# qcraftai/gedepth

Measured on AMD Instinct MI355X. Metric: training img/s (whole node), KITTI-shaped 352x1120 synthetic batches, higher is better.
Workload: dtype bf16; 1 GPU; depthformer_swint_v: DepthFormer-SwinT + GEDepth-Vanilla, 352x1120, 8 img/GPU, full train step; global_batch=8, parallelism=dp1, allreduce_dtype=fp32, layout=nhwc, window_attention=bf16 mfma, params=53516992, hip_graph=off

## Files before the change

### gedepth_amd/csrc/conv1x1_bn.hip

```cpp
#include "common.h"

#define CB_K 64
#define CB_LD 72
#define CB_GRAM (65 * CB_K)
#define CB_GRAM_WG 256

__device__ __forceinline__ int cb_row(int r, int hi) { return (r & 3) + 8 * (r >> 2) + 4 * hi; }

__global__ void __launch_bounds__(256) conv1x1_gram_k(const bf16_t* __restrict__ x, long rows, float* __restrict__ partial) {
  __shared__ __attribute__((aligned(16))) bf16_t stage_all[4][64 * CB_LD];
  __shared__ float red[CB_GRAM];
  const int lane = threadIdx.x & 63, wv = threadIdx.x >> 6, hi = lane >> 5;
  bf16_t* stage = stage_all[wv];
  ge_f32x16 acc[2][2], sum[2];
#pragma unroll
  for (int i = 0; i < 16; ++i) { acc[0][0][i] = 0.f; acc[0][1][i] = 0.f; acc[1][0][i] = 0.f; acc[1][1][i] = 0.f; sum[0][i] = 0.f; sum[1][i] = 0.f; }
  const ge_bf16x8 ones = {(__bf16)1.f, (__bf16)1.f, (__bf16)1.f, (__bf16)1.f, (__bf16)1.f, (__bf16)1.f, (__bf16)1.f, (__bf16)1.f};
  const int tr_row = hi * 8 + ((lane & 15) >> 2), tr_col = ((lane >> 4) & 1) * 16 + (lane & 3) * 4;
  const long nblk = (rows + 63) / 64;
  for (long blk = (long)blockIdx.x * 4 + wv; blk < nblk; blk += (long)gridDim.x * 4) {
    uint4 R[8];
#pragma unroll
    for (int i = 0; i < 8; ++i) {
      const int idx = i * 64 + lane;
// ... 79 lines not shown
  const int lane = threadIdx.x & 63, wv = threadIdx.x >> 6;
  cb_load_gram(gram, Ss, ss);
  const int c = blockIdx.x * 4 + wv;
  const double wi = c < Cout ? (double)bf2f(w[(long)c * CB_K + lane]) : 0.0;
  ws[wv][lane] = wi;
  __syncthreads();
  double t = 0.0;
#pragma unroll 8
  for (int j = 0; j < CB_K; ++j) t += Ss[lane * 65 + j] * ws[wv][j];
  const double mean = ge_wave_sum(wi * ss[lane]) / n;
  const double ez2 = ge_wave_sum(wi * t) / n;
  if (c >= Cout || lane != 0) return;
  double var = ez2 - mean * mean;
  if (var < 0.0) var = 0.0;
  const float rstd = (float)(1.0 / sqrt(var + (double)eps));
  save_mean[c] = (float)mean;
  save_rstd[c] = rstd;
  if (running_mean) running_mean[c] = (1.f - momentum) * running_mean[c] + momentum * (float)mean;
  if (running_var) running_var[c] = (1.f - momentum) * running_var[c] + momentum * (float)(n > 1.0 ? var * n / (n - 1.0) : var);
  const float a = gamma[c] * rstd;
  coef[c] = a;
  coef[Cout + c] = __fmaf_rn(-(float)mean, a, beta[c]);
}

#ifndef CB_EPI_GROUP
#define CB_EPI_GROUP 4
#endif
#ifdef CB_NT_STORE
#define CB_STORE16(P_, V_) { const uint4 v__ = (V_); __builtin_nontemporal_store((ge_u32x4){v__.x, v__.y, v__.z, v__.w}, (ge_u32x4*)(P_)); }
#else
#define CB_STORE16(P_, V_) *(uint4*)(P_) = (V_)
#endif
#define CB_YLD 136
template <bool HAS_POS>
__global__ void __launch_bounds__(256) conv1x1_bn_act_k(const bf16_t* __restrict__ x, const bf16_t* __restrict__ w, const float* __restrict__ coef,
                                                        const float* __restrict__ pos, bf16_t* __restrict__ y, bf16_t* __restrict__ q,
                                                        long HW, int B, int Cout, float slope) {
  __shared__ __attribute__((aligned(16))) bf16_t ytile_all[4][32 * CB_YLD];
  const int lane = threadIdx.x & 63, wv = threadIdx.x >> 6, hi = lane >> 5, n = lane & 31;
  const int cg = blockIdx.y * 4 + wv;
  if (cg * 128 >= Cout) return;
  bf16_t* ytile = ytile_all[wv];
  const int c0 = cg * 128;
  ge_bf16x8 Wf[4][4];
  float ca[4], cbv[4];
#pragma unroll
  for (int jb = 0; jb < 4; ++jb) {
#pragma unroll
    for (int s = 0; s < 4; ++s) Wf[jb][s] = *(const ge_bf16x8*)(w + (long)(c0 + jb * 32 + n) * CB_K + s * 16 + hi * 8);
    ca[jb] = coef[c0 + jb * 32 + n];
    cbv[jb] = coef[Cout + c0 + jb * 32 + n];
  }
  const int xcd = blockIdx.x & 7, wgx = gridDim.x >> 3, j0 = blockIdx.x >> 3;
  const long npt = (HW + 31) / 32;
  const long npx = npt > xcd ? (npt - xcd + 7) / 8 : 0;
  const long nq = npx * B;
  ge_bf16x8 A[4];
#define CB_LOAD_A(T_)                                                                           \
  {                                                                                             \
    const long pl_ = (T_) / B;                                                                  \
    const int b_ = (int)((T_) - pl_ * B);                                                       \
    const long p_ = (pl_ * 8 + xcd) * 32 + n;                                                   \
    const bf16_t* xr = x + ((long)b_ * HW + (p_ < HW ? p_ : HW - 1)) * CB_K + hi * 8;           \
    _Pragma("unroll") for (int s = 0; s < 4; ++s) A[s] = *(const ge_bf16x8*)(xr + s * 16);      \
  }
  if (j0 < nq) CB_LOAD_A((long)j0)
  for (long t = j0; t < nq; t += wgx) {
    const long pl = t / B;
    const int b = (int)(t - pl * B);
    const long p0 = (pl * 8 + xcd) * 32;
    ge_f32x16 acc[4];
#pragma unroll
    for (int jb = 0; jb < 4; ++jb) {
#pragma unroll
      for (int i = 0; i < 16; ++i) acc[jb][i] = 0.f;
#pragma unroll
      for (int s = 0; s < 4; ++s) acc[jb] = __builtin_amdgcn_mfma_f32_32x32x16_bf16(A[s], Wf[jb][s], acc[jb], 0, 0, 0);
    }
    if (t + wgx < nq) CB_LOAD_A(t + wgx)
    __builtin_amdgcn_wave_barrier();
#pragma unroll
    for (int jb = 0; jb < 4; ++jb)
#pragma unroll
      for (int r = 0; r < 16; ++r) {
        const float z = __fmaf_rn(acc[jb][r], ca[jb], cbv[jb]);
        ytile[cb_row(r, hi) * CB_YLD + jb * 32 + n] = f2bf_hw(z > 0.f ? z : z * slope);
      }
    __builtin_amdgcn_wave_barrier();
#pragma unroll
    for (int i0 = 0; i0 < 8; i0 += CB_EPI_GROUP) {
      float4 e0[CB_EPI_GROUP], e1[CB_EPI_GROUP];
      uint4 v[CB_EPI_GROUP];
      if (HAS_POS) {
#pragma unroll
        for (int i = 0; i < CB_EPI_GROUP; ++i) {
          const int idx = (i0 + i) * 64 + lane, tok = idx >> 4, piece = idx & 15;
          const long pr = p0 + tok < HW ? p0 + tok : HW - 1;
          const float* pp = pos + pr * Cout + c0 + piece * 8;
          e0[i] = *(const float4*)pp;
          e1[i] = *(const float4*)(pp + 4);
        }
      }
#pragma unroll
      for (int i = 0; i < CB_EPI_GROUP; ++i) {
        const int idx = (i0 + i) * 64 + lane, tok = idx >> 4, piece = idx & 15;
        v[i] = *(const uint4*)(ytile + tok * CB_YLD + piece * 8);
        if (p0 + tok < HW) CB_STORE16(y + ((long)b * HW + p0 + tok) * Cout + c0 + piece * 8, v[i]);
      }
      if (HAS_POS) {
#pragma unroll
        for (int i = 0; i < CB_EPI_GROUP; ++i) {
          const int idx = (i0 + i) * 64 + lane, tok = idx >> 4, piece = idx & 15;
          const uint32_t u[4] = {v[i].x, v[i].y, v[i].z, v[i].w};
          const float e[8] = {e0[i].x, e0[i].y, e0[i].z, e0[i].w, e1[i].x, e1[i].y, e1[i].z, e1[i].w};
          uint32_t o[4];
#pragma unroll
          for (int k = 0; k < 4; ++k) {
            const float lo = __uint_as_float(u[k] << 16) + e[2 * k], hi2 = __uint_as_float(u[k] & 0xffff0000u) + e[2 * k + 1];
            o[k] = ge_pack_bf16x2(lo, hi2);
          }
          if (p0 + tok < HW) CB_STORE16(q + ((long)b * HW + p0 + tok) * Cout + c0 + piece * 8, make_uint4(o[0], o[1], o[2], o[3]));
        }
      }
    }
  }
#undef CB_LOAD_A
}

template <bool ONE, bool TWO>
__global__ void __launch_bounds__(256) conv1x1_bn_mask_k(const bf16_t* __restrict__ dy1, long ld1, const bf16_t* __restrict__ dy2, long ld2,
                                                         const bf16_t* __restrict__ y, bf16_t* __restrict__ g, float* __restrict__ partial, int C, long R,
// ... 176 lines not shown
    }
  }
#undef CB_ROWPTR
#undef CB_LOADG
#undef CB_MMA
}

static inline bool cb_ok(int Cin, int Cout) { return Cin == CB_K && Cout > 0 && Cout % 128 == 0 && Cout <= 2048; }

extern "C" size_t ge_conv1x1_bn_workspace(int Cin, int Cout) {
  if (!cb_ok(Cin, Cout)) return 0;
  const size_t a = (size_t)CB_GRAM_WG * CB_GRAM * sizeof(float), b = (size_t)1024 * Cout * sizeof(float);
  return a > b ? a : b;
}

extern "C" int ge_conv1x1_bn_stats(const void* x, long rows, int Cin, const void* w, int Cout, const float* gamma, const float* beta,
                                   float* running_mean, float* running_var, float eps, float momentum, double* gram, float* save_mean,
                                   float* save_rstd, float* coef, void* workspace, void* stream) {
  if (!x || !w || !gamma || !beta || !gram || !save_mean || !save_rstd || !coef || !workspace || rows <= 0) return GE_ERR_BAD_ARG;
  if (!cb_ok(Cin, Cout) || (((uintptr_t)x | (uintptr_t)w) & 15)) return GE_ERR_UNSUPPORTED;
  hipStream_t s = ge_stream(stream);
  const long nblk = (rows + 63) / 64;
  const int nb = (int)(nblk < 4L * CB_GRAM_WG ? (nblk + 3) / 4 : CB_GRAM_WG);
  conv1x1_gram_k<<<nb, 256, 0, s>>>((const bf16_t*)x, rows, (float*)workspace);
  GE_LAUNCH_CHECK();
  conv1x1_partials_reduce_k<double><<<(CB_GRAM + 31) / 32, 256, 0, s>>>((const float*)workspace, nb, CB_GRAM, gram);
  GE_LAUNCH_CHECK();
  conv1x1_bn_finalize_k<<<(Cout + 3) / 4, 256, 0, s>>>(gram, (const bf16_t*)w, gamma, beta, save_mean, save_rstd, running_mean, running_var, coef,
                                                       Cout, (double)rows, eps, momentum);
  GE_LAUNCH_CHECK();
  return GE_OK;
}

extern "C" int ge_conv1x1_bn_act_fwd(const void* x, const void* w, const float* coef, const float* pos, void* y, void* q, int B, long HW, int Cin,
                                     int Cout, float slope, void* stream) {
  if (!x || !w || !coef || !y || B <= 0 || HW <= 0 || (!pos) != (!q)) return GE_ERR_BAD_ARG;
  if (!cb_ok(Cin, Cout) || (((uintptr_t)x | (uintptr_t)w | (uintptr_t)y | (uintptr_t)q | (uintptr_t)pos) & 15)) return GE_ERR_UNSUPPORTED;
  const int cus = ge_cu_count();
  if (!cus) return GE_ERR_BAD_ARG;
  hipStream_t s = ge_stream(stream);
  const long ntile = ((HW + 31) / 32) * B;
#ifndef CB_WGS_PER_CU
#define CB_WGS_PER_CU 4
#endif
  long gx = (long)cus * CB_WGS_PER_CU;
  if (gx > ntile) gx = ntile;
  gx = (gx + 7) / 8 * 8;
  const dim3 grid((unsigned)gx, (unsigned)((Cout / 128 + 3) / 4));
  if (pos) conv1x1_bn_act_k<true><<<grid, 256, 0, s>>>((const bf16_t*)x, (const bf16_t*)w, coef, pos, (bf16_t*)y, (bf16_t*)q, HW, B, Cout, slope);
  else conv1x1_bn_act_k<false><<<grid, 256, 0, s>>>((const bf16_t*)x, (const bf16_t*)w, coef, nullptr, (bf16_t*)y, nullptr, HW, B, Cout, slope);
  GE_LAUNCH_CHECK();
  return GE_OK;
}

extern "C" int ge_conv1x1_bn_bwd_mask(const void* dy1, long ld1, const void* dy2, long ld2, const void* y, void* g, float* colsum, void* workspace,
                                      long rows, int C, float slope, void* stream) {
  if ((!dy1 && !dy2) || !y || !g || !colsum || !workspace || rows <= 0 || C <= 0) return GE_ERR_BAD_ARG;
  if (C % 8 || C > 2048 || (dy1 && ld1 % 8) || (dy2 && ld2 % 8) || (((uintptr_t)dy1 | (uintptr_t)dy2 | (uintptr_t)y | (uintptr_t)g) & 15)) return GE_ERR_UNSUPPORTED;
  hipStream_t s = ge_stream(stream);
  const int lpr = C / 8;
  if (lpr > 256) return GE_ERR_UNSUPPORTED;
  const int rpi = 256 / lpr;
  const unsigned nb = ge_blocks(rows, rpi * 8, 1024);
  float* part = (float*)workspace;
#define CB_MASK(A_, B_) conv1x1_bn_mask_k<A_, B_><<<nb, 256, 0, s>>>((const bf16_t*)dy1, ld1, (const bf16_t*)dy2, ld2, (const bf16_t*)y, (bf16_t*)g, part, C, rows, lpr, rpi, slope)
  if (dy1 && dy2) CB_MASK(true, true);
  else if (dy1) CB_MASK(true, false);
  else CB_MASK(false, true);
#undef CB_MASK
  GE_LAUNCH_CHECK();
  conv1x1_partials_reduce_k<float><<<(C + 31) / 32, 256, 0, s>>>(part, (int)nb, C, colsum);
  GE_LAUNCH_CHECK();
  return GE_OK;
}

extern "C" int ge_conv1x1_bn_bwd_finalize(const float* GT, const float* colsum, const double* gram, const void* w, const float* gamma,
                                          const float* save_mean, const float* save_rstd, long rows, int Cin, int Cout, float* dgamma, float* dbeta,
                                          float* dW, void* Wd, float* c0, float* scratch, void* stream) {
  if (!GT || !colsum || !gram || !w || !gamma || !save_mean || !save_rstd || !dgamma || !dbeta || !dW || !Wd || !c0 || !scratch || rows <= 0) return GE_ERR_BAD_ARG;
  if (!cb_ok(Cin, Cout)) return GE_ERR_UNSUPPORTED;
  hipStream_t s = ge_stream(stream);
  conv1x1_bn_bwd_finalize_k<<<(Cout + 3) / 4, 256, 0, s>>>(GT, colsum, gram, (const bf16_t*)w, gamma, save_mean, save_rstd, dgamma, dbeta, dW, (bf16_t*)Wd,
                                                           scratch, scratch + Cout, Cout, (double)rows);
  GE_LAUNCH_CHECK();
  conv1x1_bn_bwd_a2_k<<<CB_K, 256, 0, s>>>((const bf16_t*)w, scratch, scratch + Cout, gram, (bf16_t*)Wd, c0, Cout, (double)rows);
// ... 23 lines not shown
```

### gedepth_amd/csrc/neck.hip

```cpp
#include "common.h"

#define NECK_TILE 64

template <typename T, bool VEC, bool DROP>
__global__ void __launch_bounds__(256) tokens_from_map_k(const T* __restrict__ map, long map_bs, const float* __restrict__ pos,
                                                         T* __restrict__ tok, long tok_bs, int C, long N, float p, float inv_keep,
                                                         uint64_t seed0, const unsigned long long* __restrict__ salt) {
  const uint64_t seed = ge_salted(seed0, salt);
  constexpr int VN = V8<T>::N, LPR = NECK_TILE / VN, RPP = 256 / LPR;
  __shared__ float tile[NECK_TILE][NECK_TILE + 1];
  const long n0 = (long)blockIdx.x * NECK_TILE;
  const int c0 = blockIdx.y * NECK_TILE, b = blockIdx.z;
  const int lane_v = (threadIdx.x % LPR) * VN, row0 = threadIdx.x / LPR;
  const T* mp = map + (long)b * map_bs;
#pragma unroll
  for (int r = row0; r < NECK_TILE; r += RPP) {
    const int c = c0 + r;
    const long n = n0 + lane_v;
    float v[VN];
    if (VEC) {
      if (c < C && n < N) {
        V8<T>::ld(mp + (long)c * N + n, v);
        if (pos) {
#pragma unroll
// ... 195 lines not shown
template <typename TI, typename TB, typename TO, bool HAS_ID>
static int scale_add_launch(const void* identity, const void* branch, const float* scale, void* out, int B, long per_sample,
                            hipStream_t s) {
  const bool vec = per_sample % 8 == 0 && al16(branch) && al16(out) && (!HAS_ID || al16(identity));
  dim3 grid(ge_blocks(vec ? per_sample / 8 : per_sample, 256 * 4, 4096), (unsigned)B);
  if (vec) scale_add_k<TI, TB, TO, HAS_ID, true><<<grid, 256, 0, s>>>((const TI*)identity, (const TB*)branch, scale, (TO*)out, per_sample);
  else scale_add_k<TI, TB, TO, HAS_ID, false><<<grid, 256, 0, s>>>((const TI*)identity, (const TB*)branch, scale, (TO*)out, per_sample);
  GE_LAUNCH_CHECK();
  return GE_OK;
}

extern "C" int ge_residual_scale_add(const void* identity, int id_dtype, const void* branch, int br_dtype, const float* scale,
                                     void* out, int B, long per_sample, void* stream) {
  if (!identity || !branch || !scale || !out || B < 0 || B > 65535 || per_sample < 0) return GE_ERR_BAD_ARG;
  if ((long)B * per_sample == 0) return GE_OK;
  hipStream_t s = ge_stream(stream);
  if (id_dtype == GE_F32 && br_dtype == GE_F32) return scale_add_launch<float, float, float, true>(identity, branch, scale, out, B, per_sample, s);
  if (id_dtype == GE_F32 && br_dtype == GE_BF16) return scale_add_launch<float, bf16_t, float, true>(identity, branch, scale, out, B, per_sample, s);
  if (id_dtype == GE_BF16 && br_dtype == GE_BF16) return scale_add_launch<bf16_t, bf16_t, bf16_t, true>(identity, branch, scale, out, B, per_sample, s);
  return GE_ERR_UNSUPPORTED;
}

extern "C" int ge_scale_rows(const void* x, int x_dtype, const float* scale, void* out, int out_dtype, int B, long per_sample,
                             void* stream) {
  if (!x || !scale || !out || B < 0 || B > 65535 || per_sample < 0) return GE_ERR_BAD_ARG;
  if ((long)B * per_sample == 0) return GE_OK;
  hipStream_t s = ge_stream(stream);
  if (x_dtype == GE_F32 && out_dtype == GE_F32) return scale_add_launch<float, float, float, false>(nullptr, x, scale, out, B, per_sample, s);
  if (x_dtype == GE_F32 && out_dtype == GE_BF16) return scale_add_launch<float, float, bf16_t, false>(nullptr, x, scale, out, B, per_sample, s);
  if (x_dtype == GE_BF16 && out_dtype == GE_BF16) return scale_add_launch<bf16_t, bf16_t, bf16_t, false>(nullptr, x, scale, out, B, per_sample, s);
  if (x_dtype == GE_BF16 && out_dtype == GE_F32) return scale_add_launch<bf16_t, bf16_t, float, false>(nullptr, x, scale, out, B, per_sample, s);
  return GE_ERR_UNSUPPORTED;
}
```

### gedepth_amd/depth/models/necks/hahi.py

```python
import os

import torch
import torch.nn as nn
import torch.nn.functional as F

from .... import kernels as K
from .... import neck_kernels as NK
from ....kernels import add_rows, concat_tokens_map, ms_deform_attn_raw, residual_dropout, tokens_from_map
from ....mmrt import bricks
from ....mmrt.bricks import BaseModule, ConvModule, build_positional_encoding, xavier_init
from ..builder import ATTENTION, NECKS


@ATTENTION.register_module()
class MultiScaleDeformableAttention(BaseModule):

    def __init__(self, embed_dims=256, num_heads=8, num_levels=4, num_points=4, im2col_step=64, dropout=0.1,
                 batch_first=False, norm_cfg=None, init_cfg=None):
        super().__init__(init_cfg)
        if embed_dims % num_heads != 0:
            raise ValueError(f'embed_dims must be divisible by num_heads, but got {embed_dims} and {num_heads}')
        if embed_dims // num_heads != 64:
            raise NotImplementedError('the HIP sampling kernel is specialised for 64 channels per head')
        self.norm_cfg, self.batch_first = norm_cfg, batch_first
        self.dropout = nn.Dropout(dropout)
        self.im2col_step = im2col_step
        self.embed_dims, self.num_levels, self.num_heads, self.num_points = embed_dims, num_levels, num_heads, num_points
        self.sampling_offsets = nn.Linear(embed_dims, num_heads * num_levels * num_points * 2)
        self.attention_weights = nn.Linear(embed_dims, num_heads * num_levels * num_points)
        self.value_proj = bricks.Linear(embed_dims, embed_dims)
        self.output_proj = bricks.Linear(embed_dims, embed_dims)
        self.init_weights()

    def init_weights(self):
        bricks.constant_init(self.sampling_offsets, 0.)
        self.sampling_offsets.bias.data = bricks.msda_offset_bias(self.num_heads, self.num_levels, self.num_points)
        bricks.constant_init(self.attention_weights, val=0., bias=0.)
        xavier_init(self.value_proj, distribution='uniform', bias=0.)
        xavier_init(self.output_proj, distribution='uniform', bias=0.)
        self._is_init = True

    def _attend(self, query, value, reference_points, spatial_shapes, key_padding_mask=None, query_shapes=None, query_order=None):
        bs, num_query, _ = query.shape
# ... 156 lines not shown
        if not levels:
            srcs, poss = [], []
            for i, ft in enumerate(feats_trans):
                h, w = shapes[i]
                pos = self.trans_positional_encoding.grid(h, w, dev).flatten(2).transpose(1, 2)
                poss.append(pos + self.level_embed[i].view(1, 1, -1))
                srcs.append((self.trans_proj[i](ft) if pre is None else self.trans_proj[i].norm_act(pre[i])).flatten(2).transpose(1, 2))
            src_flatten = torch.cat(srcs, 1)
            pos_flatten = torch.cat(poss, 1)
        if self.self_att and levels:
            q_in, v_in, id_in = NK.fan_out(src_flatten, 3) if 'neck_fanin' not in K.DISABLED else (src_flatten,) * 3
            ref = self._pixel_centres(shapes, dev).expand(bs, -1, -1, -1)
            query = NK.add_rows_levels(q_in, self._level_pos_rows(shapes, dev), self.level_embed, level_rows)
            order = (K.msda_tile_order(shapes, dev) if (os.environ.get('GE_MSDA_MM_SELF') == '1' and src_flatten.dtype == torch.bfloat16) else None)
            src = self.self_attn(query, value=v_in, identity=id_in, query_pos=None, reference_points=ref, spatial_shapes=shapes,
                                 query_shapes=shapes, query_order=order)
        elif self.self_att:
            ref = self._pixel_centres(shapes, dev).expand(bs, -1, -1, -1)
            order = (K.msda_tile_order(shapes, dev) if (os.environ.get('GE_MSDA_MM_SELF') == '1' and src_flatten.is_cuda
                                                        and src_flatten.dtype == torch.bfloat16) else None)
            src = self.self_attn(src_flatten, value=None, identity=None, query_pos=pos_flatten,
                                 reference_points=ref, spatial_shapes=shapes, query_shapes=shapes, query_order=order)
        else:
            src = src_flatten

        if levels and 'neck_fanin' not in K.DISABLED and src.dtype in (torch.float32, torch.bfloat16):
            src_value, *pieces = NK.fan_out_levels(src, level_rows)
        else:
            src_value, pieces = src, torch.split(src, level_rows, dim=1)
        h, w = feat_conv.shape[2:]
        pos_map = self.conv_positional_encoding.grid(h, w, dev) if self.cross_att else None
        query = None
        if self.training and len(self.conv_proj) == 1 and K.conv1x1_bn_act_pos_ok(self.conv_proj[0], feat_conv):
            conv_skip, query = K.conv1x1_bn_act_pos(self.conv_proj[0], feat_conv, pos_map)
        else:
            conv_skip = self.conv_proj(feat_conv)
        if self.cross_att:
            with torch.autocast('cuda', enabled=False):
                pm = pos_map.flatten(2)[0]
                w, b = self.reference_points.weight, self.reference_points.bias
                ref = torch.stack((torch.mv(pm.t(), w[0]), torch.mv(pm.t(), w[1])), -1).add(b).sigmoid()[None]
            order = self._cross_order(ref[0], shapes[0]) if (conv_skip.is_cuda and src.dtype == torch.bfloat16) else None
            ref = ref[:, :, None, :].expand(bs, -1, len(shapes), 2)
            fused = self.multi_att.forward_map(conv_skip, pos_map, src_value, ref, shapes, concat_with=feat_conv, query_order=order, query=query)
        else:
            fused = torch.cat([conv_skip, feat_conv], dim=1)
        outs = [self.conv_fusion(fused)]
        for i, (ft, piece) in enumerate(zip(feats_trans, pieces)):
            outs.append(self.trans_fusion[i](concat_tokens_map(piece, ft, tokens_first=False)))
        return tuple(outs)
```

### gedepth_amd/depth/utils/position_encoding.py

```python
import math

import torch

from ...mmrt.bricks import POSITIONAL_ENCODING, BaseModule


@POSITIONAL_ENCODING.register_module()
class SinePositionalEncoding(BaseModule):

    def __init__(self, num_feats, temperature=10000, normalize=False, scale=2 * math.pi, eps=1e-6, offset=0.,
                 init_cfg=None):
        super().__init__(init_cfg)
        if normalize:
            assert isinstance(scale, (float, int))
        self.num_feats, self.temperature, self.normalize = num_feats, temperature, normalize
        self.scale, self.eps, self.offset = scale, eps, offset
        self._cache = {}

    def grid(self, h, w, device):
        key = (h, w, str(device))
        if key not in self._cache:
            y = torch.arange(1, h + 1, dtype=torch.float32, device=device).view(h, 1).expand(h, w)
            x = torch.arange(1, w + 1, dtype=torch.float32, device=device).view(1, w).expand(h, w)
            if self.normalize:
                y = (y + self.offset) / (h + self.eps) * self.scale
                x = (x + self.offset) / (w + self.eps) * self.scale
            dim_t = torch.arange(self.num_feats, dtype=torch.float32, device=device)
            dim_t = self.temperature ** (2 * torch.div(dim_t, 2, rounding_mode='floor') / self.num_feats)
            px, py = x[:, :, None] / dim_t, y[:, :, None] / dim_t
            px = torch.stack((px[:, :, 0::2].sin(), px[:, :, 1::2].cos()), dim=3).view(h, w, -1)
            py = torch.stack((py[:, :, 0::2].sin(), py[:, :, 1::2].cos()), dim=3).view(h, w, -1)
            self._cache[key] = torch.cat((py, px), dim=2).permute(2, 0, 1).unsqueeze(0).contiguous()
        return self._cache[key]

    def forward(self, mask):
        B, h, w = mask.shape
        return self.grid(h, w, mask.device).expand(B, -1, -1, -1)
```

### gedepth_amd/kernels.py

```python
import ctypes
import os

import torch

from . import hip

_f32 = torch.float32


def _c(t):
    return t if t.is_contiguous() else t.contiguous()


class _Profiler:

    def __init__(self):
        self.on, self.records, self.stage_bytes = False, {}, {}

    def enable(self):
        self.on, self.records, self.stage_bytes = True, {}, {}
        hip.lib().ge_msda_bwd_timing(1)

    def disable(self):
        self.on = False
# ... 1443 lines not shown
        _launch(f'bn_act_bwd[{N}x{C}x{H}x{W} {_tag(x)}]', 7 * x.numel() * _es(x), 'ge_bn_act_bwd', hip.ptr(dy), hip.ptr(y), hip.ptr(x), hip.ptr(w),
                hip.ptr(stats[0]), hip.ptr(stats[1]), hip.ptr(dx), hip.ptr(dwb[0]), hip.ptr(dwb[1]), hip.ptr(ws), N, C, H * W, ctx.slope,
                hip.dtype_code(x), hip.stream())
        return dx, dwb[0], dwb[1], None, None, None, None, None


def bn_act(x, bn, slope=0.0):
    y = _BNAct.apply(x, bn.weight, bn.bias, bn.running_mean, bn.running_var, float(bn.eps), float(bn.momentum), float(slope))
    bn.num_batches_tracked.add_(1)
    return y


class _Conv1x1BNActPos(torch.autograd.Function):

    @staticmethod
    def forward(ctx, x, weight, gamma, beta, running_mean, running_var, pos_rows, eps, momentum, slope):
        from .mmrt.optim import lowp
        lib = hip.lib()
        B, Cin, H, W = x.shape
        Cout = weight.shape[0]
        HW, rows = H * W, B * H * W
        wc = lowp(weight, torch.bfloat16).detach().reshape(Cout, Cin)
        g32, b32 = _c(gamma.detach().to(_f32)), _c(beta.detach().to(_f32))
        dev = x.device
        ws = torch.empty(int(lib.ge_conv1x1_bn_workspace(Cin, Cout)), device=dev, dtype=torch.uint8)
        gram = torch.empty(65 * Cin, device=dev, dtype=torch.float64)
        stats = torch.empty(2, Cout, device=dev, dtype=_f32)
        coef = torch.empty(2, Cout, device=dev, dtype=_f32)
        y = torch.empty((B, Cout, H, W), device=dev, dtype=x.dtype, memory_format=_CL)
        q = torch.empty(B, HW, Cout, device=dev, dtype=x.dtype) if pos_rows is not None else None
        _launch(f'conv1x1_bn_stats[{B}x{Cin}->{Cout} {H}x{W}]', x.numel() * 2, 'ge_conv1x1_bn_stats', _raw_ptr(x, 'x'), rows, Cin, hip.ptr(wc), Cout,
                hip.ptr(g32), hip.ptr(b32), hip.ptr(running_mean, _f32), hip.ptr(running_var, _f32), eps, momentum, hip.ptr(gram), hip.ptr(stats[0]),
                hip.ptr(stats[1]), hip.ptr(coef), hip.ptr(ws), hip.stream())
        _launch(f'conv1x1_bn_act_fwd[{B}x{Cin}->{Cout} {H}x{W}{" +pos" if q is not None else ""}]',
                x.numel() * 2 + y.numel() * 2 * (1 + (q is not None)) + (HW * Cout * 4 if q is not None else 0), 'ge_conv1x1_bn_act_fwd',
                _raw_ptr(x, 'x'), hip.ptr(wc), hip.ptr(coef), hip.ptr(pos_rows, _f32), _raw_ptr(y, 'y'), hip.ptr(q), B, HW, Cin, Cout, slope,
                hip.stream())
        ctx.save_for_backward(x, wc, g32, stats, gram, y)
        ctx.meta = (slope, weight.dtype, gamma.dtype, beta.dtype)
        ctx.weight_ref = weight if isinstance(weight, torch.nn.Parameter) else None
        if q is None:
            return y
        return y, q

    @staticmethod
    def backward(ctx, dy, dq=None):
        x, wc, g32, stats, gram, y = ctx.saved_tensors
        slope, w_dtype, g_dtype, b_dtype = ctx.meta
        lib = hip.lib()
        B, Cin, H, W = x.shape
        Cout = wc.shape[0]
        rows = B * H * W
        dev = x.device
        ld_y = 0
        if dy is not None:
            dy = dy.to(x.dtype)
            ld_y = dy.stride(3)
            if not (dy.stride(1) == 1 and ld_y >= Cout and ld_y % 8 == 0 and dy.stride(2) == W * ld_y and dy.stride(0) == H * W * ld_y and dy.data_ptr() % 16 == 0):
                dy, ld_y = _cl(dy), Cout
        if dq is not None:
            dq = _c(dq.to(x.dtype))
        if dy is None and dq is None:
            return (None,) * 10
        ws = torch.empty(int(lib.ge_conv1x1_bn_workspace(Cin, Cout)), device=dev, dtype=torch.uint8)
        g = torch.empty(rows, Cout, device=dev, dtype=x.dtype)
        m1 = torch.empty(Cout, device=dev, dtype=_f32)
        _launch(f'conv1x1_bn_bwd_mask[{B}x{Cout} {H}x{W}]', g.numel() * 2 * (2 + (dy is not None) + (dq is not None)), 'ge_conv1x1_bn_bwd_mask',
                hip.ptr(dq), Cout, None if dy is None else _raw_ptr(dy, 'dy'), ld_y, _raw_ptr(y, 'y'), hip.ptr(g), hip.ptr(m1), hip.ptr(ws), rows,
                Cout, slope, hip.stream())
        GT = torch.zeros(Cout, Cin, device=dev, dtype=_f32)
        _launch(f'conv1x1_wgrad[{B}x{Cin}->{Cout} {H}x{W}]', (x.numel() + g.numel()) * 2 + GT.numel() * 4, 'ge_conv1x1_nhwc_wgrad', _raw_ptr(x, 'x'),
                hip.ptr(g), hip.ptr(GT), rows, Cin, Cout, hip.GE_BF16, hip.stream())
        small = torch.empty(2 * Cout + Cout * Cin + 2 * Cout, device=dev, dtype=_f32)
        dgamma, dbeta, dW, scratch = small[:Cout], small[Cout:2 * Cout], small[2 * Cout:2 * Cout + Cout * Cin].view(Cout, Cin), small[2 * Cout + Cout * Cin:]
        Wd = torch.empty(Cin, Cout + Cin, device=dev, dtype=x.dtype)
        c0 = torch.empty(Cin, device=dev, dtype=_f32)
        hip.call('ge_conv1x1_bn_bwd_finalize', hip.ptr(GT), hip.ptr(m1), hip.ptr(gram), hip.ptr(wc), hip.ptr(g32), hip.ptr(stats[0]),
                 hip.ptr(stats[1]), rows, Cin, Cout, hip.ptr(dgamma), hip.ptr(dbeta), hip.ptr(dW), hip.ptr(Wd), hip.ptr(c0), hip.ptr(scratch),
                 hip.stream())
        dx = None
        if ctx.needs_input_grad[0]:
            dx = torch.empty_like(x)
            _launch(f'conv1x1_bn_dgrad[{B}x{Cout}->{Cin} {H}x{W}]', (g.numel() + 2 * x.numel()) * 2, 'ge_conv1x1_bn_dgrad', hip.ptr(g),
                    _raw_ptr(x, 'x'), hip.ptr(Wd), hip.ptr(c0), _raw_ptr(dx, 'dx'), rows, Cin, Cout, hip.stream())
        dw = dW.view(Cout, Cin, 1, 1)
        if ctx.weight_ref is not None:
            from .mmrt.optim import grad_into_arena
            dw = grad_into_arena(ctx.weight_ref, dw, w_dtype)
        else:
            dw = dw.to(w_dtype)
        return dx, dw, dgamma.to(g_dtype), dbeta.to(b_dtype), None, None, None, None, None, None


def conv1x1_bn_act_pos_ok(block, x):
    conv, bn = block.conv, block.norm
    return ('conv1x1_bn' not in DISABLED and x.is_cuda and x.dtype == torch.bfloat16 and type(conv) is torch.nn.Conv2d and conv.kernel_size == (1, 1)
            and conv.stride == (1, 1) and conv.padding == (0, 0) and conv.groups == 1 and conv.bias is None and conv.in_channels == 64
            and conv.out_channels % 128 == 0 and conv.out_channels <= 1024 and conv.weight.dtype == _f32
            and torch.is_autocast_enabled() and torch.get_autocast_dtype('cuda') == torch.bfloat16
            and block._fused_bn_slope() is not None and _is_cl(x) and x.data_ptr() % 16 == 0)


def conv1x1_bn_act_pos(block, x, pos=None):
    bn = block.norm
    slope = float(block._fused_bn_slope())
    pos_rows = _pos_rows(pos) if pos is not None else None
    out = _Conv1x1BNActPos.apply(x, block.conv.weight, bn.weight, bn.bias, bn.running_mean, bn.running_var, pos_rows, float(bn.eps), float(bn.momentum), slope)
    bn.num_batches_tracked.add_(1)
    return out if pos is not None else (out, None)


class _BiasAct(torch.autograd.Function):

    @staticmethod
    def forward(ctx, x, bias, slope):
        ctx.cl = _cl_ok(x)
        assert x.dim() == 4 and (x.is_contiguous() or ctx.cl), 'bias_act works in place on a dense NCHW / channels-last conv output'
        N, C, H, W = x.shape
        b = _c(bias.detach().to(_f32))
        if ctx.cl:
            _launch(f'bias_act_nhwc_fwd[{N}x{C}x{H}x{W} {_tag(x)}]', 2 * x.numel() * _es(x), 'ge_bias_act_nhwc_fwd', _raw_ptr(x, 'x'), hip.ptr(b),
                    N * H * W, C, slope, hip.dtype_code(x), hip.stream())
            ctx.mark_dirty(x)
            ctx.save_for_backward(x)
            ctx.slope = slope
            return x
        _launch(f'bias_act_fwd[{N}x{C}x{H}x{W} {_tag(x)}]', 2 * x.numel() * _es(x), 'ge_bias_act_fwd', hip.ptr(x, name='x'), hip.ptr(b), N, C, H * W,
                slope, hip.dtype_code(x), hip.stream())
        ctx.mark_dirty(x)
        ctx.save_for_backward(x)
        ctx.slope = slope
        return x

    @staticmethod
    def backward(ctx, dy):
        y, = ctx.saved_tensors
        N, C, H, W = y.shape
        dx = torch.empty_like(y)
        if ctx.cl:
# ... 282 lines not shown
```

### gedepth_amd/neck_kernels.py

```python
import ctypes

import torch

from . import hip
from .kernels import _c, _cl_ok, _es, _f32, _launch, _tag

MAX_LEVELS = 8
_WS = {}


def _starts(level_rows, n_levels=None):
    n_levels = len(level_rows) if n_levels is None else n_levels
    if not 1 <= len(level_rows) <= n_levels <= MAX_LEVELS or any(r < 0 for r in level_rows):
        raise ValueError(f'a level table takes 1 .. {MAX_LEVELS} levels of non-negative size, got {tuple(level_rows)} for {n_levels} levels')
    starts, acc = [0], 0
    for l in range(n_levels):
        acc += int(level_rows[l]) if l < len(level_rows) else 0
        starts.append(acc)
    return (ctypes.c_long * len(starts))(*starts), n_levels, acc


def _workspace(device, C, K):
    key = (device, hip.stream(), C, K)
    ws = _WS.get(key)
# ... 158 lines not shown

    @staticmethod
    def backward(ctx, *gs):
        gs = [g for g in gs if g is not None]
        if not gs:
            return None, None
        return (gs[0] if len(gs) == 1 else token_grad_sum(gs)), None


def fan_out(x, n):
    assert 1 <= n <= 3
    return _FanOut.apply(x, n)


class _FanOutLevels(torch.autograd.Function):

    @staticmethod
    def forward(ctx, x, level_rows):
        ctx.set_materialize_grads(False)
        ctx.meta = (tuple(x.shape), x.dtype, x.device, level_rows)
        return (x.view_as(x), *x.split(list(level_rows), 1))

    @staticmethod
    def backward(ctx, g, *parts):
        (B, N, C), dtype, device, level_rows = ctx.meta
        if all(p is None for p in parts):
            return g, None
        parts = [torch.zeros(B, n, C, device=device, dtype=dtype) if p is None else p for p, n in zip(parts, level_rows)]
        return token_grad_sum([] if g is None else [g], parts), None


def fan_out_levels(x, level_rows):
    return _FanOutLevels.apply(x, tuple(int(r) for r in level_rows))
```

### include/gedepth_neck.h

```cpp
#ifndef GEDEPTH_NECK_H
#define GEDEPTH_NECK_H

#include <stddef.h>
#include <stdint.h>

#ifdef __cplusplus
extern "C" {
#endif

#define GE_NECK_MAX_LEVELS 8

int ge_bn_act_nhwc_fwd_rows(const void* x, const float* gamma, const float* beta, void* y, long rows_per_image, long image_stride,
                            float* save_mean, float* save_rstd, float* running_mean, float* running_var, void* workspace, long rows, int C,
                            float eps, float momentum, float slope, int dtype, void* stream);
int ge_bn_act_nhwc_bwd_rows(const void* dy, long rows_per_image, long image_stride, const void* x, const float* gamma, const float* beta,
                            const float* save_mean, const float* save_rstd, void* dx, float* dgamma, float* dbeta, void* workspace, long rows,
                            int C, float slope, int dtype, void* stream);

int ge_add_rows_levels(const void* x, const float* pos, const float* emb, void* out, int B, long N, int C, const long* level_starts,
                       int n_levels, int dtype, void* stream);

int ge_level_colsum(const void* x, int B, long N, int C, const long* level_starts, int n_levels, float* out, void* workspace, int dtype,
                    void* stream);

int ge_token_grad_sum(const void* a0, const void* a1, const void* a2, const void* const* parts, const long* pitch, const long* col,
                      const long* level_starts, int n_parts, void* out, int B, long N, int C, int dtype, void* stream);

#ifdef __cplusplus
}
#endif
#endif
```

Before: 178.4 img/s.

## Exploit separable sine positional encoding in neck reference points and pos-add

The sine positional map is split into a per-row table (y features) and a per-column table (x features). The reference-point projection becomes two small per-row and per-column dot products plus a sigmoid, replacing a matvec over the full H*W x 2F map, and its backward uses the same factorisation with fp64 reductions. The fused conv1x1+BN+act kernel now reads positional values from these two tables instead of a dense HW x Cout fp32 pos array, which cuts memory traffic in its epilogue. The cost is extra kernel launches and an integer divide per token in the epilogue.

```diff
diff --git a/gedepth_amd/csrc/conv1x1_bn.hip b/gedepth_amd/csrc/conv1x1_bn.hip
--- a/gedepth_amd/csrc/conv1x1_bn.hip
+++ b/gedepth_amd/csrc/conv1x1_bn.hip
@@ -135,10 +135,10 @@
 #define CB_STORE16(P_, V_) *(uint4*)(P_) = (V_)
 #endif
 #define CB_YLD 136
-template <bool HAS_POS>
+template <bool HAS_POS, bool SEP>
 __global__ void __launch_bounds__(256) conv1x1_bn_act_k(const bf16_t* __restrict__ x, const bf16_t* __restrict__ w, const float* __restrict__ coef,
-                                                        const float* __restrict__ pos, bf16_t* __restrict__ y, bf16_t* __restrict__ q,
-                                                        long HW, int B, int Cout, float slope) {
+                                                        const float* __restrict__ pos, const float* __restrict__ px, int Wm, int F,
+                                                        bf16_t* __restrict__ y, bf16_t* __restrict__ q, long HW, int B, int Cout, float slope) {
   __shared__ __attribute__((aligned(16))) bf16_t ytile_all[4][32 * CB_YLD];
   const int lane = threadIdx.x & 63, wv = threadIdx.x >> 6, hi = lane >> 5, n = lane & 31;
   const int cg = blockIdx.y * 4 + wv;
@@ -199,7 +199,14 @@
         for (int i = 0; i < CB_EPI_GROUP; ++i) {
           const int idx = (i0 + i) * 64 + lane, tok = idx >> 4, piece = idx & 15;
           const long pr = p0 + tok < HW ? p0 + tok : HW - 1;
-          const float* pp = pos + pr * Cout + c0 + piece * 8;
+          const float* pp;
+          if (SEP) {
+            const unsigned row = (unsigned)pr / (unsigned)Wm, col = (unsigned)pr - row * (unsigned)Wm;
+            const int c = c0 + piece * 8;
+            pp = c < F ? pos + (long)row * F + c : px + (long)col * F + (c - F);
+          } else {
+            pp = pos + pr * Cout + c0 + piece * 8;
+          }
           e0[i] = *(const float4*)pp;
           e1[i] = *(const float4*)(pp + 4);
         }
@@ -442,9 +449,8 @@
   return GE_OK;
 }
 
-extern "C" int ge_conv1x1_bn_act_fwd(const void* x, const void* w, const float* coef, const float* pos, void* y, void* q, int B, long HW, int Cin,
-                                     int Cout, float slope, void* stream) {
-  if (!x || !w || !coef || !y || B <= 0 || HW <= 0 || (!pos) != (!q)) return GE_ERR_BAD_ARG;
+static int cb_act_fwd(const void* x, const void* w, const float* coef, const float* pos, const float* px, int Wm, void* y, void* q, int B, long HW,
+                      int Cin, int Cout, float slope, void* stream) {
   if (!cb_ok(Cin, Cout) || (((uintptr_t)x | (uintptr_t)w | (uintptr_t)y | (uintptr_t)q | (uintptr_t)pos) & 15)) return GE_ERR_UNSUPPORTED;
   const int cus = ge_cu_count();
   if (!cus) return GE_ERR_BAD_ARG;
@@ -457,10 +463,24 @@
   if (gx > ntile) gx = ntile;
   gx = (gx + 7) / 8 * 8;
   const dim3 grid((unsigned)gx, (unsigned)((Cout / 128 + 3) / 4));
-  if (pos) conv1x1_bn_act_k<true><<<grid, 256, 0, s>>>((const bf16_t*)x, (const bf16_t*)w, coef, pos, (bf16_t*)y, (bf16_t*)q, HW, B, Cout, slope);
-  else conv1x1_bn_act_k<false><<<grid, 256, 0, s>>>((const bf16_t*)x, (const bf16_t*)w, coef, nullptr, (bf16_t*)y, nullptr, HW, B, Cout, slope);
+  if (px) conv1x1_bn_act_k<true, true><<<grid, 256, 0, s>>>((const bf16_t*)x, (const bf16_t*)w, coef, pos, px, Wm, Cout / 2, (bf16_t*)y, (bf16_t*)q, HW, B, Cout, slope);
+  else if (pos) conv1x1_bn_act_k<true, false><<<grid, 256, 0, s>>>((const bf16_t*)x, (const bf16_t*)w, coef, pos, nullptr, 0, 0, (bf16_t*)y, (bf16_t*)q, HW, B, Cout, slope);
+  else conv1x1_bn_act_k<false, false><<<grid, 256, 0, s>>>((const bf16_t*)x, (const bf16_t*)w, coef, nullptr, nullptr, 0, 0, (bf16_t*)y, nullptr, HW, B, Cout, slope);
   GE_LAUNCH_CHECK();
   return GE_OK;
+}
+
+extern "C" int ge_conv1x1_bn_act_fwd(const void* x, const void* w, const float* coef, const float* pos, void* y, void* q, int B, long HW, int Cin,
+                                     int Cout, float slope, void* stream) {
+  if (!x || !w || !coef || !y || B <= 0 || HW <= 0 || (!pos) != (!q)) return GE_ERR_BAD_ARG;
+  return cb_act_fwd(x, w, coef, pos, nullptr, 0, y, q, B, HW, Cin, Cout, slope, stream);
+}
+
+extern "C" int ge_conv1x1_bn_act_fwd_sep(const void* x, const void* w, const float* coef, const float* py, const float* px, void* y, void* q, int B,
+                                         int H, int Wm, int Cin, int Cout, float slope, void* stream) {
+  if (!x || !w || !coef || !y || !q || !py || !px || B <= 0 || H <= 0 || Wm <= 0 || (long)H * Wm > 2147483647L) return GE_ERR_BAD_ARG;
+  if (((uintptr_t)px) & 15) return GE_ERR_UNSUPPORTED;
+  return cb_act_fwd(x, w, coef, py, px, Wm, y, q, B, (long)H * Wm, Cin, Cout, slope, stream);
 }
 
 extern "C" int ge_conv1x1_bn_bwd_mask(const void* dy1, long ld1, const void* dy2, long ld2, const void* y, void* g, float* colsum, void* workspace,
diff --git a/gedepth_amd/csrc/neck.hip b/gedepth_amd/csrc/neck.hip
--- a/gedepth_amd/csrc/neck.hip
+++ b/gedepth_amd/csrc/neck.hip
@@ -251,3 +251,168 @@
   if (x_dtype == GE_BF16 && out_dtype == GE_F32) return scale_add_launch<bf16_t, bf16_t, float, false>(nullptr, x, scale, out, B, per_sample, s);
   return GE_ERR_UNSUPPORTED;
 }
+
+#define RP_ROWS 4
+
+template <int N, typename V>
+__device__ __forceinline__ void rp_block_tree(V* red, int t) {
+#pragma unroll
+  for (int s = 128; s >= N; s >>= 1) {
+    if (t < s) red[t] += red[t + s];
+    __syncthreads();
+  }
+}
+
+template <typename A>
+__global__ void __launch_bounds__(256) ref_points_tables_k(const float* __restrict__ py, const float* __restrict__ px, const float* __restrict__ w,
+                                                           A* __restrict__ t, int H, int F) {
+  __shared__ A red[2][256];
+  const int i = blockIdx.x, tid = threadIdx.x;
+  const float* p = i < H ? py + (long)i * F : px + (long)(i - H) * F;
+  const float* w0 = w + (i < H ? 0 : F);
+  A a0 = 0, a1 = 0;
+  for (int c = tid; c < F; c += 256) {
+    const A v = p[c];
+    a0 = fma(v, (A)w0[c], a0);
+    a1 = fma(v, (A)w0[2 * F + c], a1);
+  }
+  red[0][tid] = a0;
+  red[1][tid] = a1;
+  __syncthreads();
+  rp_block_tree<1>(red[0], tid);
+  rp_block_tree<1>(red[1], tid);
+  if (tid < 2) t[2 * (long)i + tid] = red[tid][0];
+}
+
+__device__ __forceinline__ float rp_sigmoid(float z) { return 1.f / (1.f + expf(-z)); }
+
+__global__ void __launch_bounds__(256) ref_points_fwd_k(const float* __restrict__ t, const float* __restrict__ b, float* __restrict__ ref, int H, int W) {
+  const long j = (long)blockIdx.x * 256 + threadIdx.x;
+  if (j >= 2L * H * W) return;
+  const int k = (int)(j & 1);
+  const long pos = j >> 1;
+  const int row = (int)(pos / W), col = (int)(pos - (long)row * W);
+  ref[j] = rp_sigmoid(t[2 * row + k] + t[2 * (H + col) + k] + b[k]);
+}
+
+__global__ void __launch_bounds__(256) ref_points_sums_k(const float* __restrict__ d_ref, const double* __restrict__ t, const float* __restrict__ b,
+                                                         double* __restrict__ gy, double* __restrict__ colpart, int H, int W) {
+  __shared__ double red[256];
+  const int tid = threadIdx.x, r0 = blockIdx.x * RP_ROWS, W2 = 2 * W;
+  double rowacc[RP_ROWS];
+#pragma unroll
+  for (int r = 0; r < RP_ROWS; ++r) rowacc[r] = 0.0;
+  const double bk = b[tid & 1];
+  for (int j = tid; j < W2; j += 256) {
+    double colacc = 0.0;
+    const double txb = t[2 * H + j] + bk;
+#pragma unroll
+    for (int r = 0; r < RP_ROWS; ++r) {
+      if (r0 + r < H) {
+        const long e = (long)(r0 + r) * W2 + j;
+        const double ez = exp(-fabs(t[2 * (r0 + r) + (tid & 1)] + txb));
+        const double g = (double)d_ref[e] * ez / ((1.0 + ez) * (1.0 + ez));
+        colacc += g;
+        rowacc[r] += g;
+      }
+    }
+    colpart[(long)blockIdx.x * W2 + j] = colacc;
+  }
+#pragma unroll
+  for (int r = 0; r < RP_ROWS; ++r) {
+    red[tid] = rowacc[r];
+    __syncthreads();
+    rp_block_tree<2>(red, tid);
+    if (tid < 2 && r0 + r < H) gy[2 * (r0 + r) + tid] = red[tid];
+    __syncthreads();
+  }
+}
+
+__global__ void __launch_bounds__(256) ref_points_fold_k(const double* __restrict__ colpart, const double* __restrict__ gy, double* __restrict__ gx,
+                                                         float* __restrict__ d_b, int H, int W, int nrb) {
+  __shared__ double red[256];
+  const int tid = threadIdx.x, W2 = 2 * W;
+  if (blockIdx.x + 1 < gridDim.x) {
+    const int j = blockIdx.x * 256 + tid;
+    if (j >= W2) return;
+    double a = 0.0;
+    for (int x = 0; x < nrb; ++x) a += colpart[(long)x * W2 + j];
+    gx[j] = a;
+    return;
+  }
+  double a = 0.0;
+  for (int j = tid; j < 2 * H; j += 256) a += gy[j];
+  red[tid] = a;
+  __syncthreads();
+  rp_block_tree<2>(red, tid);
+  if (tid < 2) d_b[tid] = (float)red[tid];
+}
+
+__global__ void __launch_bounds__(256) ref_points_dw_k(const float* __restrict__ py, const float* __restrict__ px, const double* __restrict__ gy,
+                                                       const double* __restrict__ gx, float* __restrict__ d_w, int H, int W, int F) {
+  __shared__ double red[2][8][32];
+  const int lane = threadIdx.x & 31, grp = threadIdx.x >> 5;
+  const int c = blockIdx.x * 32 + lane;
+  const bool live = c < 2 * F, top = c < F;
+  const float* tab = top ? py : px;
+  const double* gs = top ? gy : gx;
+  const int n = top ? H : W, cc = top ? c : c - F;
+  double a0 = 0.0, a1 = 0.0;
+  for (int i = grp; live && i < n; i += 8) {
+    const double v = tab[(long)i * F + cc];
+    a0 = fma(gs[2 * i], v, a0);
+    a1 = fma(gs[2 * i + 1], v, a1);
+  }
+  red[0][grp][lane] = a0;
+  red[1][grp][lane] = a1;
+  __syncthreads();
+  if (threadIdx.x < 64) {
+    const int k = threadIdx.x >> 5;
+    double sum = 0.0;
+#pragma unroll
+    for (int g = 0; g < 8; ++g) sum += red[k][g][lane];
+    if (live) d_w[(long)k * 2 * F + c] = (float)sum;
+  }
+}
+
+static inline bool rp_args_ok(int H, int W, int F) { return H > 0 && W > 0 && F > 0 && F <= (1 << 20) && (long)H * W <= (1L << 30) && (long)H + W <= (1L << 30); }
+static inline long rp_row_blocks(int H) { return ((long)H + RP_ROWS - 1) / RP_ROWS; }
+
+extern "C" size_t ge_ref_points_sep_workspace(int H, int W) {
+  if (H <= 0 || W <= 0) return 0;
+  return (size_t)(4L * (H + W) + rp_row_blocks(H) * 2L * W) * sizeof(double);
+}
+
+extern "C" int ge_ref_points_sep_fwd(const float* py, const float* px, const float* w, const float* b, float* ref, void* workspace, int H, int W,
+                                     int F, void* stream) {
+  if (!py || !px || !w || !b || !ref || !workspace || !rp_args_ok(H, W, F)) return GE_ERR_BAD_ARG;
+  if ((uintptr_t)workspace & 7) return GE_ERR_UNSUPPORTED;
+  hipStream_t s = ge_stream(stream);
+  float* t = (float*)workspace;
+  ref_points_tables_k<float><<<(unsigned)(H + W), 256, 0, s>>>(py, px, w, t, H, F);
+  GE_LAUNCH_CHECK();
+  ref_points_fwd_k<<<(unsigned)((2L * H * W + 255) / 256), 256, 0, s>>>(t, b, ref, H, W);
+  GE_LAUNCH_CHECK();
+  return GE_OK;
+}
+
+extern "C" int ge_ref_points_sep_bwd(const float* d_ref, const float* py, const float* px, const float* w, const float* b, float* d_w, float* d_b,
+                                     void* workspace, int H, int W, int F, void* stream) {
+  if (!d_ref || !py || !px || !w || !b || !d_w || !d_b || !workspace || !rp_args_ok(H, W, F)) return GE_ERR_BAD_ARG;
+  if ((uintptr_t)workspace & 7) return GE_ERR_UNSUPPORTED;
+  hipStream_t s = ge_stream(stream);
+  const long nrb = rp_row_blocks(H);
+  double* t = (double*)workspace;
+  double* gy = t + 2L * (H + W);
+  double* gx = gy + 2L * H;
+  double* colpart = gx + 2L * W;
+  ref_points_tables_k<double><<<(unsigned)(H + W), 256, 0, s>>>(py, px, w, t, H, F);
+  GE_LAUNCH_CHECK();
+  ref_points_sums_k<<<(unsigned)nrb, 256, 0, s>>>(d_ref, t, b, gy, colpart, H, W);
+  GE_LAUNCH_CHECK();
+  ref_points_fold_k<<<(unsigned)((2L * W + 255) / 256 + 1), 256, 0, s>>>(colpart, gy, gx, d_b, H, W, (int)nrb);
+  GE_LAUNCH_CHECK();
+  ref_points_dw_k<<<(unsigned)((2L * F + 31) / 32), 256, 0, s>>>(py, px, gy, gx, d_w, H, W, F);
+  GE_LAUNCH_CHECK();
+  return GE_OK;
+}
diff --git a/gedepth_amd/depth/models/necks/hahi.py b/gedepth_amd/depth/models/necks/hahi.py
--- a/gedepth_amd/depth/models/necks/hahi.py
+++ b/gedepth_amd/depth/models/necks/hahi.py
@@ -9,6 +9,7 @@
 from ....kernels import add_rows, concat_tokens_map, ms_deform_attn_raw, residual_dropout, tokens_from_map
 from ....mmrt import bricks
 from ....mmrt.bricks import BaseModule, ConvModule, build_positional_encoding, xavier_init
+from ...utils.position_encoding import SinePositionalEncoding
 from ..builder import ATTENTION, NECKS
 
 
@@ -231,14 +232,19 @@
         pos_map = self.conv_positional_encoding.grid(h, w, dev) if self.cross_att else None
         query = None
         if self.training and len(self.conv_proj) == 1 and K.conv1x1_bn_act_pos_ok(self.conv_proj[0], feat_conv):
-            conv_skip, query = K.conv1x1_bn_act_pos(self.conv_proj[0], feat_conv, pos_map)
+            tabs = (self.conv_positional_encoding.tables(h, w, dev) if (pos_map is not None and 'pos_tables' not in K.DISABLED
+                                                                        and isinstance(self.conv_positional_encoding, SinePositionalEncoding)) else None)
+            conv_skip, query = K.conv1x1_bn_act_pos(self.conv_proj[0], feat_conv, pos_map, tables=tabs)
         else:
             conv_skip = self.conv_proj(feat_conv)
         if self.cross_att:
-            with torch.autocast('cuda', enabled=False):
-                pm = pos_map.flatten(2)[0]
-                w, b = self.reference_points.weight, self.reference_points.bias
-                ref = torch.stack((torch.mv(pm.t(), w[0]), torch.mv(pm.t(), w[1])), -1).add(b).sigmoid()[None]
+            rw, rb = self.reference_points.weight, self.reference_points.bias
+            if NK.ref_points_sep_ok(self.conv_positional_encoding, rw, rb):
+                ref = NK.ref_points_sep(*self.conv_positional_encoding.tables(h, w, dev), rw, rb)[None]
+            else:
+                with torch.autocast('cuda', enabled=False):
+                    pm = pos_map.flatten(2)[0]
+                    ref = torch.stack((torch.mv(pm.t(), rw[0]), torch.mv(pm.t(), rw[1])), -1).add(rb).sigmoid()[None]
             order = self._cross_order(ref[0], shapes[0]) if (conv_skip.is_cuda and src.dtype == torch.bfloat16) else None
             ref = ref[:, :, None, :].expand(bs, -1, len(shapes), 2)
             fused = self.multi_att.forward_map(conv_skip, pos_map, src_value, ref, shapes, concat_with=feat_conv, query_order=order, query=query)
diff --git a/gedepth_amd/depth/utils/position_encoding.py b/gedepth_amd/depth/utils/position_encoding.py
--- a/gedepth_amd/depth/utils/position_encoding.py
+++ b/gedepth_amd/depth/utils/position_encoding.py
@@ -33,6 +33,13 @@
             self._cache[key] = torch.cat((py, px), dim=2).permute(2, 0, 1).unsqueeze(0).contiguous()
         return self._cache[key]
 
+    def tables(self, h, w, device):
+        key = ('tables', h, w, str(device))
+        if key not in self._cache:
+            g, f = self.grid(h, w, device)[0], self.num_feats
+            self._cache[key] = (g[:f, :, 0].t().contiguous(), g[f:, 0, :].t().contiguous())
+        return self._cache[key]
+
     def forward(self, mask):
         B, h, w = mask.shape
         return self.grid(h, w, mask.device).expand(B, -1, -1, -1)
diff --git a/gedepth_amd/kernels.py b/gedepth_amd/kernels.py
--- a/gedepth_amd/kernels.py
+++ b/gedepth_amd/kernels.py
@@ -1499,10 +1499,16 @@
         _launch(f'conv1x1_bn_stats[{B}x{Cin}->{Cout} {H}x{W}]', x.numel() * 2, 'ge_conv1x1_bn_stats', _raw_ptr(x, 'x'), rows, Cin, hip.ptr(wc), Cout,
                 hip.ptr(g32), hip.ptr(b32), hip.ptr(running_mean, _f32), hip.ptr(running_var, _f32), eps, momentum, hip.ptr(gram), hip.ptr(stats[0]),
                 hip.ptr(stats[1]), hip.ptr(coef), hip.ptr(ws), hip.stream())
-        _launch(f'conv1x1_bn_act_fwd[{B}x{Cin}->{Cout} {H}x{W}{" +pos" if q is not None else ""}]',
-                x.numel() * 2 + y.numel() * 2 * (1 + (q is not None)) + (HW * Cout * 4 if q is not None else 0), 'ge_conv1x1_bn_act_fwd',
-                _raw_ptr(x, 'x'), hip.ptr(wc), hip.ptr(coef), hip.ptr(pos_rows, _f32), _raw_ptr(y, 'y'), hip.ptr(q), B, HW, Cin, Cout, slope,
-                hip.stream())
+        if isinstance(pos_rows, tuple):
+            py, px = pos_rows
+            assert tuple(py.shape) == (H, Cout // 2) and tuple(px.shape) == (W, Cout // 2)
+            from .neck_kernels import conv1x1_bn_act_fwd_tables
+            conv1x1_bn_act_fwd_tables(x, wc, coef, py, px, y, q, slope)
+        else:
+            _launch(f'conv1x1_bn_act_fwd[{B}x{Cin}->{Cout} {H}x{W}{" +pos" if q is not None else ""}]',
+                    x.numel() * 2 + y.numel() * 2 * (1 + (q is not None)) + (HW * Cout * 4 if q is not None else 0), 'ge_conv1x1_bn_act_fwd',
+                    _raw_ptr(x, 'x'), hip.ptr(wc), hip.ptr(coef), hip.ptr(pos_rows, _f32), _raw_ptr(y, 'y'), hip.ptr(q), B, HW, Cin, Cout, slope,
+                    hip.stream())
         ctx.save_for_backward(x, wc, g32, stats, gram, y)
         ctx.meta = (slope, weight.dtype, gamma.dtype, beta.dtype)
         ctx.weight_ref = weight if isinstance(weight, torch.nn.Parameter) else None
@@ -1568,10 +1574,10 @@
             and block._fused_bn_slope() is not None and _is_cl(x) and x.data_ptr() % 16 == 0)
 
 
-def conv1x1_bn_act_pos(block, x, pos=None):
+def conv1x1_bn_act_pos(block, x, pos=None, tables=None):
     bn = block.norm
     slope = float(block._fused_bn_slope())
-    pos_rows = _pos_rows(pos) if pos is not None else None
+    pos_rows = None if pos is None else tables if tables is not None else _pos_rows(pos)
     out = _Conv1x1BNActPos.apply(x, block.conv.weight, bn.weight, bn.bias, bn.running_mean, bn.running_var, pos_rows, float(bn.eps), float(bn.momentum), slope)
     bn.num_batches_tracked.add_(1)
     return out if pos is not None else (out, None)
diff --git a/gedepth_amd/neck_kernels.py b/gedepth_amd/neck_kernels.py
--- a/gedepth_amd/neck_kernels.py
+++ b/gedepth_amd/neck_kernels.py
@@ -214,3 +214,51 @@
 
 def fan_out_levels(x, level_rows):
     return _FanOutLevels.apply(x, tuple(int(r) for r in level_rows))
+
+
+class _RefPointsSep(torch.autograd.Function):
+
+    @staticmethod
+    def forward(ctx, py, px, w, b):
+        (H, F), W = py.shape, px.shape[0]
+        assert px.shape[1] == F and tuple(w.shape) == (2, 2 * F) and tuple(b.shape) == (2,)
+        w32, b32 = _c(w.detach().to(_f32)), _c(b.detach().to(_f32))
+        ref = torch.empty(H * W, 2, device=py.device, dtype=_f32)
+        ws = torch.empty(int(hip.lib().ge_ref_points_sep_workspace(H, W)), device=py.device, dtype=torch.uint8)
+        _launch(f'ref_points_sep_fwd[{H}x{W}x{2 * F}]', (H + W) * F * 4 + ref.numel() * 4, 'ge_ref_points_sep_fwd', hip.ptr(py, _f32, 'py'),
+                hip.ptr(px, _f32, 'px'), hip.ptr(w32), hip.ptr(b32), hip.ptr(ref), hip.ptr(ws), H, W, F, hip.stream())
+        ctx.save_for_backward(py, px, w32, b32)
+        ctx.dtypes = (w.dtype, b.dtype)
+        return ref
+
+    @staticmethod
+    def backward(ctx, d_ref):
+        py, px, w32, b32 = ctx.saved_tensors
+        (H, F), W = py.shape, px.shape[0]
+        d_ref = _c(d_ref.to(_f32))
+        d_w = torch.empty(2, 2 * F, device=py.device, dtype=_f32)
+        d_b = torch.empty(2, device=py.device, dtype=_f32)
+        ws = torch.empty(int(hip.lib().ge_ref_points_sep_workspace(H, W)), device=py.device, dtype=torch.uint8)
+        _launch(f'ref_points_sep_bwd[{H}x{W}x{2 * F}]', d_ref.numel() * 4 + 2 * (H + W) * F * 4, 'ge_ref_points_sep_bwd', hip.ptr(d_ref), hip.ptr(py),
+                hip.ptr(px), hip.ptr(w32), hip.ptr(b32), hip.ptr(d_w), hip.ptr(d_b), hip.ptr(ws), H, W, F, hip.stream())
+        return None, None, d_w.to(ctx.dtypes[0]), d_b.to(ctx.dtypes[1])
+
+
+def ref_points_sep_ok(encoding, w, b):
+    from .depth.utils.position_encoding import SinePositionalEncoding
+    from .kernels import DISABLED
+    return ('ref_tables' not in DISABLED and isinstance(encoding, SinePositionalEncoding) and w.is_cuda and w.dtype == _f32 and b.dtype == _f32
+            and tuple(w.shape) == (2, 2 * encoding.num_feats))
+
+
+def ref_points_sep(py, px, w, b):
+    return _RefPointsSep.apply(py, px, w, b)
+
+
+def conv1x1_bn_act_fwd_tables(x, wc, coef, py, px, y, q, slope):
+    from .kernels import _raw_ptr
+    B, Cin, H, W = x.shape
+    Cout = wc.shape[0]
+    _launch(f'conv1x1_bn_act_fwd[{B}x{Cin}->{Cout} {H}x{W} +pos tables]', x.numel() * 2 + y.numel() * 4 + (H + W) * Cout * 2,
+            'ge_conv1x1_bn_act_fwd_sep', _raw_ptr(x, 'x'), hip.ptr(wc), hip.ptr(coef), hip.ptr(py, _f32, 'py'), hip.ptr(px, _f32, 'px'),
+            _raw_ptr(y, 'y'), hip.ptr(q), B, H, W, Cin, Cout, slope, hip.stream())
diff --git a/include/gedepth_neck.h b/include/gedepth_neck.h
--- a/include/gedepth_neck.h
+++ b/include/gedepth_neck.h
@@ -26,6 +26,15 @@
 int ge_token_grad_sum(const void* a0, const void* a1, const void* a2, const void* const* parts, const long* pitch, const long* col,
                       const long* level_starts, int n_parts, void* out, int B, long N, int C, int dtype, void* stream);
 
+size_t ge_ref_points_sep_workspace(int H, int W);
+int ge_ref_points_sep_fwd(const float* py, const float* px, const float* w, const float* b, float* ref, void* workspace, int H, int W, int F,
+                          void* stream);
+int ge_ref_points_sep_bwd(const float* d_ref, const float* py, const float* px, const float* w, const float* b, float* d_w, float* d_b,
+                          void* workspace, int H, int W, int F, void* stream);
+
+int ge_conv1x1_bn_act_fwd_sep(const void* x, const void* w, const float* coef, const float* py, const float* px, void* y, void* q, int B, int H,
+                              int Wm, int Cin, int Cout, float slope, void* stream);
+
 #ifdef __cplusplus
 }
 #endif
```

Result: no change. 180.1 img/s, median of 6 (+1.0%).
